# MoeinSorkhei/APLA

Measured on NVIDIA B200. Metric: ViT-B/14 APLA fine-tune images/sec/GPU at 1/2/4/8 B200; % bf16 tensor roofline, higher is better.
Workload: dtype bf16

## Files before the change

apla_b200/csrc/attention.cu:

```cuda
#include <cstdlib>

#include "common.cuh"
#include "kernels.cuh"
#include "ptx.cuh"

namespace apla {

namespace {

__global__ void attn_delta_kernel(const __nv_bfloat16* __restrict__ dout, const __nv_bfloat16* __restrict__ out,
                                  float* __restrict__ delta, size_t n_chunks) {
  const size_t i = size_t(blockIdx.x) * blockDim.x + threadIdx.x;
  float acc = 0.f;
  if (i < n_chunks) {
    const uint4 a = __ldg(reinterpret_cast<const uint4*>(dout) + i);
    const uint4 b = __ldg(reinterpret_cast<const uint4*>(out) + i);
    const uint32_t aw[4] = {a.x, a.y, a.z, a.w}, bw[4] = {b.x, b.y, b.z, b.w};
#pragma unroll
    for (int t = 0; t < 4; ++t) acc += bf16_lo(aw[t]) * bf16_lo(bw[t]) + bf16_hi(aw[t]) * bf16_hi(bw[t]);
  }
  acc += __shfl_xor_sync(0xffffffffu, acc, 1);
  acc += __shfl_xor_sync(0xffffffffu, acc, 2);
  acc += __shfl_xor_sync(0xffffffffu, acc, 4);
  if ((threadIdx.x & 7) == 0 && i < n_chunks) delta[i >> 3] = acc;
}

}

int attn_fwd(const void* qkv, void* out, float* lse, const int* cu_seqlens, int num_seqs, int max_seqlen,
             int total_tokens, int H,
             float scale, cudaStream_t stream) {
  APLA_CHECK(num_seqs > 0 && max_seqlen > 0 && H > 0, "attn_fwd: empty problem");
  if (attn_fused_supported(max_seqlen))
    return attn_fwd_sr(qkv, out, lse, cu_seqlens, num_seqs, max_seqlen, total_tokens, H, scale, stream);
  return attn_fwd_tc(qkv, out, lse, cu_seqlens, num_seqs, max_seqlen, total_tokens, H, scale, stream);
}

int attn_bwd(const void* qkv, const void* out, const void* dout, const float* lse, float* delta, void* dqkv,
             const int* cu_seqlens, int num_seqs, int max_seqlen, int total_tokens, int H, float scale,
             cudaStream_t stream) {
  APLA_CHECK(num_seqs > 0 && max_seqlen > 0 && H > 0, "attn_bwd: empty problem");
  if (out != nullptr) {
    const size_t n_chunks = size_t(total_tokens) * H * 8;
    attn_delta_kernel<<<(unsigned)((n_chunks + 255) / 256), 256, 0, stream>>>(
        reinterpret_cast<const __nv_bfloat16*>(dout), reinterpret_cast<const __nv_bfloat16*>(out), delta, n_chunks);
    APLA_CUDA(cudaGetLastError());
    count_launch();
  }
  static const bool v1 = [] { const char* e = getenv("APLA_ATTN_BWD_V1"); return e && atoi(e) != 0; }();
  if (!v1 && attn_bwd2_supported(max_seqlen))
    return attn_bwd2(qkv, dout, lse, delta, dqkv, cu_seqlens, num_seqs, max_seqlen, total_tokens, H, scale, stream);
  if (attn_fused_supported(max_seqlen))
    return attn_bwd_fused(qkv, dout, lse, delta, dqkv, cu_seqlens, num_seqs, max_seqlen, total_tokens, H, scale, stream);
  return attn_bwd_tc(qkv, dout, lse, delta, dqkv, cu_seqlens, num_seqs, max_seqlen, total_tokens, H, scale, stream);
}

}
```

apla_b200/csrc/attention_bwd2.cu:

```cuda
#include <cstdlib>

#include "common.cuh"
#include "kernels.cuh"
#include "ptx.cuh"

namespace apla {
namespace afb {

constexpr float LOG2E = 1.4426950408889634f;
constexpr int NT_MAX = 256;
constexpr int CW = 64;
constexpr int MAX_CHUNKS = NT_MAX / CW;
constexpr int kThreads = 640;
constexpr uint32_t RES_BYTES = NT_MAX * 128;
constexpr uint32_t TILE_BYTES = 128 * 128;
constexpr uint32_t OFF_Q = 0, OFF_DO = RES_BYTES, OFF_KV = 2 * RES_BYTES;
constexpr uint32_t OFF_DS = OFF_KV + 4 * TILE_BYTES;
constexpr uint32_t OFF_STAT = OFF_DS + 4 * TILE_BYTES;
constexpr uint32_t OFF_VEC = OFF_STAT + 2 * NT_MAX * 4;
constexpr uint32_t OFF_COL = OFF_VEC + 2 * 4 * 64 * 4;
constexpr uint32_t OFF_ROW = OFF_COL + 2 * 2 * NT_MAX * 4;
constexpr uint32_t OFF_PART = OFF_ROW + 2 * 2 * 128 * 4;
constexpr uint32_t OFF_BAR = OFF_PART + 4 * 3 * 64 * 4;
constexpr uint32_t SMEM_BYTES = OFF_BAR + 512 + 1024;
constexpr uint32_t TM_DQ = 0, TM_DK = 128, TM_DV = 192, TM_S = 256, TM_DP = 384, TM_COLS = 512;
static_assert(SMEM_BYTES <= 227 * 1024, "shared memory budget");

constexpr int REG_LAUNCH = 96;
constexpr int REG_WG0 = 56, REG_COMPUTE = 136, REG_EPI = 80, REG_HELP = 72;
static_assert(REG_WG0 + 2 * REG_COMPUTE + REG_EPI + REG_HELP <= 5 * REG_LAUNCH, "setmaxnreg budget exceeds the CTA's pool");

__device__ __forceinline__ void tmem_st_32x16(uint32_t taddr, const uint32_t (&v)[16]) {
  asm volatile(
      "tcgen05.st.sync.aligned.32x32b.x16.b32 [%0], {%1, %2, %3, %4, %5, %6, %7, %8, %9, %10, %11, %12, %13, %14, %15, %16};" ::
          "r"(taddr),
      "r"(v[0]), "r"(v[1]), "r"(v[2]), "r"(v[3]), "r"(v[4]), "r"(v[5]), "r"(v[6]), "r"(v[7]), "r"(v[8]), "r"(v[9]),
      "r"(v[10]), "r"(v[11]), "r"(v[12]), "r"(v[13]), "r"(v[14]), "r"(v[15])
      : "memory");
}
__device__ __forceinline__ void tmem_st_wait() { asm volatile("tcgen05.wait::st.sync.aligned;" ::: "memory"); }
__device__ __forceinline__ bool mbar_test(uint64_t* bar, uint32_t parity) {
  uint32_t ok;
  asm volatile(
      "{\n\t.reg .pred p;\n\t"
      "mbarrier.test_wait.parity.shared::cta.b64 p, [%1], %2;\n\t"
      "selp.u32 %0, 1, 0, p;\n\t}"
      : "=r"(ok)
      : "r"(smem_u32(bar)), "r"(parity)
      : "memory");
  return ok != 0;
}

constexpr uint32_t DESC_HI = (1024u >> 4) | (1u << 14) | (2u << 29);
constexpr uint32_t DESC_LO_K = (16u >> 4) << 16;
constexpr uint32_t DESC_LO_MN = (16384u >> 4) << 16;

__device__ __forceinline__ void umma_ss(uint32_t tmem_d, uint32_t a_lo, uint32_t b_lo, uint32_t idesc, uint32_t accumulate) {
  asm volatile(
      "{\n\t.reg .pred p;\n\t.reg .b64 da, db;\n\t"
      "setp.ne.b32 p, %4, 0;\n\t"
      "mov.b64 da, {%1, %5};\n\t"
      "mov.b64 db, {%2, %5};\n\t"
      "tcgen05.mma.cta_group::1.kind::f16 [%0], da, db, %3, p;\n\t}" ::"r"(tmem_d),
      "r"(a_lo), "r"(b_lo), "r"(idesc), "r"(accumulate), "r"(DESC_HI)
      : "memory");
}
__device__ __forceinline__ void umma_ts(uint32_t tmem_d, uint32_t tmem_a, uint32_t b_lo, uint32_t idesc, uint32_t accumulate) {
  asm volatile(
      "{\n\t.reg .pred p;\n\t.reg .b64 db;\n\t"
      "setp.ne.b32 p, %4, 0;\n\t"
      "mov.b64 db, {%2, %5};\n\t"
      "tcgen05.mma.cta_group::1.kind::f16 [%0], [%1], db, %3, p;\n\t}" ::"r"(tmem_d),
      "r"(tmem_a), "r"(b_lo), "r"(idesc), "r"(accumulate), "r"(DESC_HI)
      : "memory");
}

#ifdef APLA_AFB_DEBUG
__device__ __forceinline__ void wait_tag(uint64_t* bar, uint32_t parity, int tag) {
  uint32_t spins = 0;
  while (!mbar_try_wait(bar, parity)) {
    if (++spins > (1u << 16)) {
      if ((threadIdx.x & 31) == 0)
        printf("afb HANG cta %d warp %d tag %d parity %u\n", blockIdx.x, threadIdx.x >> 5, tag, parity);
// ... 108 lines not shown
    b0 = fmaf(bf16_lo(xb.z), q1.x, b0);
    b1 = fmaf(bf16_hi(xb.z), q1.y, b1);
    a0 = fmaf(bf16_lo(xa.w), p1.z, a0);
    a1 = fmaf(bf16_hi(xa.w), p1.w, a1);
    b0 = fmaf(bf16_lo(xb.w), q1.z, b0);
    b1 = fmaf(bf16_hi(xb.w), q1.w, b1);
  }
  da = a0 + a1;
  db = b0 + b1;
}
__device__ __forceinline__ float dot_vec64(uint32_t a, uint32_t b) {
  float s0 = 0.f, s1 = 0.f;
#pragma unroll 4
  for (int u = 0; u < 16; ++u) {
    const float4 x = lds_f4(a + 16 * u);
    const float4 y = lds_f4(b + 16 * u);
    s0 = fmaf(x.x, y.x, s0);
    s1 = fmaf(x.y, y.y, s1);
    s0 = fmaf(x.z, y.z, s0);
    s1 = fmaf(x.w, y.w, s1);
  }
  return s0 + s1;
}

__device__ __forceinline__ void drain_row64(uint32_t taddr, float mul, bool rank1, float coef, uint32_t vec,
                                            __nv_bfloat16* dst, bool store) {
  uint32_t pk[32];
#pragma unroll
  for (int c = 0; c < 2; ++c) {
    uint32_t ov[32];
    tmem_ld_32x32(taddr + c * 32, ov);
    tmem_ld_wait();
    if (rank1) {
#pragma unroll
      for (int i = 0; i < 8; ++i) {
        const float4 v = lds_f4(vec + (c * 32 + 4 * i) * 4);
        ov[4 * i + 0] = __float_as_uint(fmaf(coef, v.x, __uint_as_float(ov[4 * i + 0])));
        ov[4 * i + 1] = __float_as_uint(fmaf(coef, v.y, __uint_as_float(ov[4 * i + 1])));
        ov[4 * i + 2] = __float_as_uint(fmaf(coef, v.z, __uint_as_float(ov[4 * i + 2])));
        ov[4 * i + 3] = __float_as_uint(fmaf(coef, v.w, __uint_as_float(ov[4 * i + 3])));
      }
    }
#pragma unroll
    for (int i = 0; i < 16; ++i)
      pk[c * 16 + i] = pack_bf16(__uint_as_float(ov[2 * i]) * mul, __uint_as_float(ov[2 * i + 1]) * mul);
  }
  if (store) {
    uint4* d4 = reinterpret_cast<uint4*>(dst);
#pragma unroll
    for (int j = 0; j < 8; ++j) d4[j] = make_uint4(pk[4 * j], pk[4 * j + 1], pk[4 * j + 2], pk[4 * j + 3]);
  }
}

__global__ void __launch_bounds__(kThreads, 1)
attn_bwd2_kernel(const __grid_constant__ Maps maps, const __nv_bfloat16* __restrict__ qkv,
                 const __nv_bfloat16* __restrict__ dout, const float* __restrict__ lse, const float* __restrict__ delta,
                 __nv_bfloat16* __restrict__ dqkv, const int* __restrict__ cu_seqlens, int n_fixed, int H, int G,
                 float scale, int ablate) {
#ifndef APLA_AFB_ABLATE
  ablate = 0;
#endif
  extern __shared__ uint8_t smem_raw[];
  uint8_t* smem = reinterpret_cast<uint8_t*>((reinterpret_cast<uintptr_t>(smem_raw) + 1023) & ~uintptr_t(1023));
  uint64_t* bars = reinterpret_cast<uint64_t*>(smem + OFF_BAR);
  uint64_t* qdo_full = bars;
  uint64_t* qdo_empty = bars + 4;
  uint64_t* kv_full = bars + 8;
  uint64_t* kv_empty = bars + 10;
  uint64_t* s_full = bars + 12;
  uint64_t* s_free = bars + 14;
  uint64_t* dp_full = bars + 16;
  uint64_t* pd_full = bars + 18;
  uint64_t* ds_empty = bars + 20;
  uint64_t* acc_full = bars + 22;
  uint64_t* acc_empty = bars + 23;
  uint64_t* dq_full = bars + 24;
  uint64_t* dq_empty = bars + 25;
  uint64_t* hrow_full = bars + 26;
  uint64_t* hrow_empty = bars + 28;
  uint64_t* hcol_full = bars + 30;
  uint64_t* hcol_empty = bars + 32;
  uint64_t* pk_full = bars + 34;
  uint32_t* tmem_slot = reinterpret_cast<uint32_t*>(bars + 38);

  const int warp = __shfl_sync(0xffffffffu, threadIdx.x >> 5, 0), lane = threadIdx.x & 31;
  const Problem prob{cu_seqlens, n_fixed, H, G, (ablate & 2) != 0};
  const int D = H * 64;

  if (warp == 0 && lane == 0) {
    tma_prefetch_desc(&maps.qkv64);
    tma_prefetch_desc(&maps.qkv16);
    tma_prefetch_desc(&maps.do64);
    tma_prefetch_desc(&maps.do16);
    for (int i = 0; i < MAX_CHUNKS; ++i) {
      mbar_init(&qdo_full[i], 2);
      mbar_init(&qdo_empty[i], 4);
    }
    for (int i = 0; i < 2; ++i) {
      mbar_init(&kv_full[i], 1);
      mbar_init(&kv_empty[i], 4);
      mbar_init(&s_full[i], 1);
      mbar_init(&s_free[i], 4);
      mbar_init(&dp_full[i], 1);
      mbar_init(&pd_full[i], 4);
      mbar_init(&ds_empty[i], 1);
      mbar_init(&hrow_full[i], 1);
      mbar_init(&hrow_empty[i], 4);
      mbar_init(&hcol_full[i], 1);
      mbar_init(&hcol_empty[i], 4);
    }
    for (int i = 0; i < 4; ++i) mbar_init(&pk_full[i], 4);
    mbar_init(acc_full, 2);
    mbar_init(acc_empty, 4);
    mbar_init(dq_full, 1);
    mbar_init(dq_empty, 4);
    fence_barrier_init();
  }
  if (warp == 1) {
    tmem_alloc<1>(tmem_slot, TM_COLS);
    tmem_relinquish<1>();
  }
  tc_fence_before();
  __syncthreads();
  tc_fence_after();
  const uint32_t tmem = __shfl_sync(0xffffffffu, *tmem_slot, 0);
#ifdef APLA_AFB_PROF
  uint32_t prof[20];
#pragma unroll
  for (int i = 0; i < 20; ++i) prof[i] = 0;
  const long long prof_t0 = clock64();
#endif

#ifdef APLA_AFB_TRACE
  __shared__ long long tr_buf[6][200];
  __shared__ int tr_n[6];
  __shared__ long long tr_t0s;
  if (threadIdx.x == 0) {
    for (int i = 0; i < 6; ++i) tr_n[i] = 0;
    tr_t0s = clock64();
  }
  __syncthreads();
  const long long tr_t0 = tr_t0s;
#define TR(role, ev, arg)                                                                              \
  do {                                                                                                 \
    if (blockIdx.x == 0 && lane == 0 && tr_n[role] < 200)                                              \
      tr_buf[role][tr_n[role]++] = ((clock64() - tr_t0) << 16) | ((long long)(ev) << 8) | ((arg) & 255); \
  } while (0)
#else
#define TR(role, ev, arg)
#endif
  const uint32_t sb = smem_u32(smem);
  const uint32_t a_sl = sb + OFF_STAT, a_sd = a_sl + NT_MAX * 4;
  const uint32_t a_vec = sb + OFF_VEC;
  const uint32_t a_col = sb + OFF_COL;
  const uint32_t a_row = sb + OFF_ROW;

  if (warp < 4) {
    reg_dealloc<REG_WG0>();
    const bool leader = elect_one();
    const uint32_t q_lo = smem_u32(smem + OFF_Q) >> 4, do_lo = smem_u32(smem + OFF_DO) >> 4;
    const uint32_t kv_lo = smem_u32(smem + OFF_KV) >> 4, ds_lo = smem_u32(smem + OFF_DS) >> 4;
    if (warp == 0) {
      auto load_rows = [&](uint8_t* dst, const CUtensorMap* m64, const CUtensorMap* m16, uint64_t* bar, int col, int row,
                           int rows) {
        int r = 0;
        for (; r + 64 <= rows; r += 64) tma_load_2d(dst + r * 128, m64, bar, col, row + r);
// ... 109 lines not shown
        bool ok = true;
        if (w.jt == 0) ok = mbar_test(&qdo_full[w.j], (w.qpar >> w.j) & 1);
        if (ok && w.j == 0) ok = mbar_test(&kv_full[w.ts & 1], (w.ts >> 1) & 1);
        return __all_sync(0xffffffffu, ok) != 0;
      };
      Walk pc, dc;
      pc.init(prob);
      dc = pc;
      while (!dc.done(prob)) {
        while (!pc.done(prob) && pc.c <= dc.c) {
          wait_operands(pc);
          issue_dp(pc);
          pc.next_chunk(prob);
        }
        if (!pc.done(prob) && pc.c - dc.c < 2 && operands_ready(pc)) {
          tc_fence_after();
          issue_dp(pc);
          pc.next_chunk(prob);
        }
        const int slot = dc.ts & 1;
        WAIT(&pd_full[dc.c & 1], (dc.c >> 1) & 1, 8);
        if (dc.j == 0) WAIT(acc_empty, (dc.ts & 1) ^ 1, 9);
        tc_fence_after();
        const int n_k = (dc.valid_cols() + 15) >> 4;
        const uint32_t b_do = DESC_LO_MN + do_lo + dc.j * (CW * 128 >> 4);
        const uint32_t t_p = tmem + TM_DP + (dc.c & 1) * CW;
        TR(0, 4, dc.c);
        if (leader) {
#pragma unroll
          for (int kk = 0; kk < CW / 16; ++kk)
            if (kk < n_k) umma_ts(tmem + TM_DV, t_p + kk * 8, b_do + kk * 128, idesc_acc, (dc.j > 0 || kk > 0) ? 1u : 0u);
          if (dc.last_tile()) umma_commit(&qdo_empty[dc.j]);
          if (dc.last_chunk()) {
            umma_commit(acc_full);
            umma_commit(&kv_empty[slot]);
          }
        }
        __syncwarp();
        dc.next_chunk(prob);
        while (!pc.done(prob) && pc.c - dc.c < 2 && operands_ready(pc)) {
          tc_fence_after();
          issue_dp(pc);
          pc.next_chunk(prob);
        }
      }
    } else {
      const uint32_t idesc_acc = make_idesc_bf16(128, 64, 0, 1);
      const uint32_t idesc_dq = make_idesc_bf16(128, 64, 1, 1);
      Walk a;
      a.init(prob);
      while (!a.done(prob)) {
        const int slot = a.ts & 1;
        WAIT(&pk_full[a.c & 3], (a.c >> 2) & 1, 10);
        if (a.j == 0) WAIT(acc_empty, (a.ts & 1) ^ 1, 11);
        tc_fence_after();
        const int n_k = (a.valid_cols() + 15) >> 4;
        const int tq = a.tq();
        const uint32_t a_ds = DESC_LO_K + ds_lo + ((tq & 1) * 2 + (a.j & 1)) * (TILE_BYTES >> 4);
        const uint32_t b_q = DESC_LO_MN + q_lo + a.j * (CW * 128 >> 4);
        TR(0, 5, a.c);
        if (leader) {
#pragma unroll
          for (int kk = 0; kk < CW / 16; ++kk)
            if (kk < n_k && !(ablate & 16)) umma_ss(tmem + TM_DK, a_ds + 2 * kk, b_q + kk * 128, idesc_acc, (a.j > 0 || kk > 0) ? 1u : 0u);
          if (a.last_tile()) umma_commit(&qdo_empty[a.j]);
        }
        __syncwarp();
        if ((a.j & 1) || a.last_chunk()) {
          const int t = a.j >> 1;
          if (a.jt == 0 && t == 0) {
            WAIT(dq_empty, (a.gi & 1) ^ 1, 12);
            tc_fence_after();
          }
          const int n_kk = (a.valid_keys() + 15) >> 4;
          const uint32_t a_pair = DESC_LO_MN + ds_lo + (tq & 1) * (2 * TILE_BYTES >> 4);
          const uint32_t b_k = DESC_LO_MN + kv_lo + slot * (2 * TILE_BYTES >> 4);
          if (leader) {
#pragma unroll
            for (int kk = 0; kk < 8; ++kk)
              if (kk < n_kk && !(ablate & 16))
                umma_ss(tmem + TM_DQ + t * 64, a_pair + kk * 128, b_k + kk * 128, idesc_dq, (a.jt > 0 || kk > 0) ? 1u : 0u);
            umma_commit(&ds_empty[tq & 1]);
          }
          __syncwarp();
        }
        if (a.last_chunk()) {
          if (leader) {
            umma_commit(acc_full);
            umma_commit(&kv_empty[slot]);
            if (a.last_tile()) umma_commit(dq_full);
          }
          __syncwarp();
        }
        a.next_chunk(prob);
      }
    }
  } else if (warp < 12) {
    reg_alloc<REG_COMPUTE>();
    const int wg = (warp - 4) >> 2;
    const int quad = warp & 3;
    const int row = quad * 32 + lane;
    const uint32_t lane_addr = tmem + (uint32_t(quad * 32) << 16);
    const float sl2 = scale * LOG2E;
    const uint32_t sw = uint32_t(row & 7);
    Walk k;
    k.init(prob);
    while (!k.done(prob)) {
// ... 71 lines not shown
            pk[2 * i + 1] = pack_bf16(__uint_as_float(p0[4 * i + 2]) * (__uint_as_float(dv[4 * i + 2]) - d.z),
                                      __uint_as_float(p0[4 * i + 3]) * (__uint_as_float(dv[4 * i + 3]) - d.w));
          }
          CP(12);
          WAIT(&ds_empty[tq & 1], ((tq >> 1) & 1) ^ 1, 9);
          CP(19);
#pragma unroll
          for (int u = 0; u < 4; ++u) {
            uint4 val = make_uint4(pk[4 * u], pk[4 * u + 1], pk[4 * u + 2], pk[4 * u + 3]);
            if (!key_ok) val = make_uint4(0u, 0u, 0u, 0u);
            sts_u4(panel_row + ((uint32_t(u) ^ sw) << 4), val);
          }
#pragma unroll
          for (int i = 0; i < 16; ++i) pk[i] = pack_bf16(__uint_as_float(p0[2 * i]), __uint_as_float(p0[2 * i + 1]));
          tmem_st_32x16(t_dp, pk);
        }
        if (two) {
          uint32_t dv[32], pk[16];
          tmem_ld_32x32(t_dp + 32, dv);
          tmem_ld_wait();
#pragma unroll
          for (int i = 0; i < 8; ++i) {
            const float4 d = lds_f4(sD + 128 + 16 * i);
            pk[2 * i] = pack_bf16(__uint_as_float(p1[4 * i + 0]) * (__uint_as_float(dv[4 * i + 0]) - d.x),
                                  __uint_as_float(p1[4 * i + 1]) * (__uint_as_float(dv[4 * i + 1]) - d.y));
            pk[2 * i + 1] = pack_bf16(__uint_as_float(p1[4 * i + 2]) * (__uint_as_float(dv[4 * i + 2]) - d.z),
                                      __uint_as_float(p1[4 * i + 3]) * (__uint_as_float(dv[4 * i + 3]) - d.w));
          }
#pragma unroll
          for (int u = 0; u < 4; ++u) {
            uint4 val = make_uint4(pk[4 * u], pk[4 * u + 1], pk[4 * u + 2], pk[4 * u + 3]);
            if (!key_ok) val = make_uint4(0u, 0u, 0u, 0u);
            sts_u4(panel_row + ((uint32_t(4 + u) ^ sw) << 4), val);
          }
#pragma unroll
          for (int i = 0; i < 16; ++i) pk[i] = pack_bf16(__uint_as_float(p1[2 * i]), __uint_as_float(p1[2 * i + 1]));
          tmem_st_32x16(t_dp + 16, pk);
        }
        CP(13);
        tmem_st_wait();
        fence_proxy_async_smem();
        CP(14);
      }
      tc_fence_before();
      __syncwarp();
      if (lane == 0) {
        mbar_arrive(&pd_full[k.c & 1]);
        mbar_arrive(&pk_full[k.c & 3]);
      }
      if (quad == 0) TR(1 + wg, 5, k.c);
      k.next_chunk(prob);
    }
  } else if (warp < 16) {
    reg_dealloc<REG_EPI>();
    const int quad = warp & 3;
    const int row = quad * 32 + lane;
    const uint32_t lane_addr = tmem + (uint32_t(quad * 32) << 16);
    Walk k;
    k.init(prob);
    while (!k.done(prob)) {
      const int par = k.gi & 1, slot = k.ts & 1;
      const bool odd = k.odd != 0;
      const uint32_t vecs = a_vec + par * 1024;
      if (quad == 0) TR(3, 1, k.ts);
      WAIT(acc_full, k.ts & 1, 10);
      if (quad == 0) TR(3, 2, k.ts);
      tc_fence_after();
      WAIT(&hrow_full[slot], (k.ts >> 1) & 1, 11);
      if (quad == 0) TR(3, 3, k.ts);
      {
        const int r = k.jt * 128 + row;
        const bool ok = r < k.nt;
        __nv_bfloat16* base = dqkv + size_t(k.row_start + (ok ? r : 0)) * (3 * D) + k.h * 64;
        float cp = 0.f, cds = 0.f;
        if (odd) {
          cp = lds_f32(a_row + (slot * 256 + row) * 4);
          cds = lds_f32(a_row + (slot * 256 + 128 + row) * 4);
        }
        __syncwarp();
        if (lane == 0) mbar_arrive(&hrow_empty[slot]);
        if (!(ablate & 4))
        drain_row64(lane_addr + TM_DK, scale, odd, cds, vecs, base + D, ok);
        {
          uint32_t pk[32];
#pragma unroll
          for (int c = 0; c < 2; ++c) {
            uint32_t ov[32];
            if (!(ablate & 4)) {
              tmem_ld_32x32(lane_addr + TM_DV + c * 32, ov);
              tmem_ld_wait();
            }
            if (c == 1) {
              tc_fence_before();
              __syncwarp();
              if (lane == 0) mbar_arrive(acc_empty);
            }
            if (odd) {
#pragma unroll
              for (int i = 0; i < 8; ++i) {
                const float4 v = lds_f4(vecs + (192 + c * 32 + 4 * i) * 4);
                ov[4 * i + 0] = __float_as_uint(fmaf(cp, v.x, __uint_as_float(ov[4 * i + 0])));
                ov[4 * i + 1] = __float_as_uint(fmaf(cp, v.y, __uint_as_float(ov[4 * i + 1])));
                ov[4 * i + 2] = __float_as_uint(fmaf(cp, v.z, __uint_as_float(ov[4 * i + 2])));
                ov[4 * i + 3] = __float_as_uint(fmaf(cp, v.w, __uint_as_float(ov[4 * i + 3])));
              }
            }
#pragma unroll
            for (int i = 0; i < 16; ++i)
              pk[c * 16 + i] = pack_bf16(__uint_as_float(ov[2 * i]), __uint_as_float(ov[2 * i + 1]));
          }
          if (ok && !(ablate & 4)) {
            uint4* d4 = reinterpret_cast<uint4*>(base + 2 * D);
#pragma unroll
            for (int j = 0; j < 8; ++j) d4[j] = make_uint4(pk[4 * j], pk[4 * j + 1], pk[4 * j + 2], pk[4 * j + 3]);
          }
        }
      }
      if (k.last_tile()) {
        WAIT(dq_full, k.gi & 1, 12);
        tc_fence_after();
        WAIT(&hcol_full[par], (k.gi >> 1) & 1, 13);
        for (int t = 0; t < k.ntiles; ++t) {
          const int r = t * 128 + row;
          const bool ok = r < k.nt;
          __nv_bfloat16* base = dqkv + size_t(k.row_start + (ok ? r : 0)) * (3 * D) + k.h * 64;
          const float cq = odd ? lds_f32(a_col + (par * 512 + 256 + r) * 4) : 0.f;
          if (!(ablate & 4))
          drain_row64(lane_addr + TM_DQ + t * 64, scale, odd, cq, vecs + 64 * 4, base, ok);
        }
        tc_fence_before();
        __syncwarp();
        if (lane == 0) {
          mbar_arrive(dq_empty);
          mbar_arrive(&hcol_empty[par]);
        }
      }
      if (quad == 0) TR(3, 4, k.ts);
      const int ts0 = k.ts;
      while (!k.done(prob) && k.ts == ts0) k.next_chunk(prob);
    }
  } else {
    reg_dealloc<REG_HELP>();
    const int e = threadIdx.x - 512;
    const int dpair = e & 31, part = e >> 5;
    const float sl2 = scale * LOG2E;
    const uint32_t a_part = sb + OFF_PART;
    const uint32_t dp_off = (uint32_t(dpair & 3) << 2);
#ifdef APLA_AFB_PROF
    long long hp_t = clock64();
#define HP(i) do { const long long _n = clock64(); prof[i] += uint32_t(_n - hp_t); hp_t = _n; } while (0)
#else
#define HP(i)
#endif
    Walk k;
    k.init(prob);
    int ts = 0;
    while (!k.done(prob)) {
      HP(0);
      const int par = k.gi & 1;
      const bool odd = k.odd != 0;
      const int o = k.nt;
      const uint32_t vecs = a_vec + par * 1024, cols = a_col + par * 2048;
      WAIT(&hcol_empty[par], ((k.gi >> 1) & 1) ^ 1, 14);
      float lse2_o = 0.f, delta_o = 0.f;
      if (odd) {
        const int v = e >> 5;
        const size_t tok = size_t(k.row_start + o);
        const __nv_bfloat16* src = v < 3 ? qkv + tok * (3 * D) + v * D + k.h * 64 : dout + tok * D + k.h * 64;
        const uint32_t w2 = __ldg(reinterpret_cast<const uint32_t*>(src) + lane);
        sts_f32(vecs + (v * 64 + 2 * lane) * 4, bf16_lo(w2));
        sts_f32(vecs + (v * 64 + 2 * lane + 1) * 4, bf16_hi(w2));
        lse2_o = __ldg(lse + tok * H + k.h) * LOG2E;
        delta_o = __ldg(delta + tok * H + k.h);
      }
      HP(1);
      for (int j = 0; j < k.nchunks; ++j) WAIT(&qdo_full[j], (k.qpar >> j) & 1, 15);
      asm volatile("bar.sync 2, 128;" ::: "memory");
      HP(0);
      float p_oo = 0.f, ds_oo = 0.f;
      float ko0 = 0.f, ko1 = 0.f, vo0 = 0.f, vo1 = 0.f;
      if (odd) {
        const float s_oo = dot_vec64(vecs, vecs + 64 * 4), dp_oo = dot_vec64(vecs + 192 * 4, vecs + 128 * 4);
        p_oo = exp2f(fmaf(s_oo, sl2, -lse2_o));
        ds_oo = p_oo * (dp_oo - delta_o);
#pragma unroll
        for (int qq = 0; qq < 2; ++qq) {
          const int q = e + 128 * qq;
          float p = 0.f, ds = 0.f;
          if (q < k.nt) {
            float s, dp;
            dot2_row64(sb + OFF_Q + q * 128, sb + OFF_DO + q * 128, q, vecs + 64 * 4, vecs + 128 * 4, s, dp);
            p = exp2f(fmaf(s, sl2, -lds_f32(a_sl + q * 4)));
            ds = p * (dp - lds_f32(a_sd + q * 4));
          }
          sts_f32(cols + q * 4, p);
// ... 87 lines not shown
      k.next_group(prob);
    }
  }
#ifdef APLA_AFB_PROF
  if (blockIdx.x == 0 && lane == 0 && (warp == 4 || warp == 8 || warp == 5))
    printf("afb compute warp %d phases: S-load %u exps %u dP-load+dS-half0 %u stores+half1 %u st-wait+fence %u\n", warp, prof[10], prof[11],
           prof[12], prof[13], prof[14]);
  if (blockIdx.x == 0 && lane == 0 && warp == 16)
    printf("afb helper phases: other/waits %u vec-load %u col %u dk-loop %u tile-dots %u dq-loop %u finalize %u\n", prof[0], prof[1],
           prof[2], prof[3], prof[4], prof[5], prof[6]);
  if (blockIdx.x == 0 && lane == 0 && (warp <= 2 || (warp & 3) == 0) && warp != 16)
    printf("afb prof warp %2d total %lld | kv_empty %u qdo_empty %u acc_empty %u dq_empty %u qdo_empty(st) %u | qdo_full %u s_full %u "
           "dp_full %u ds_empty %u | acc_full %u hrow_full %u dq_full %u hcol_full %u | hcol_empty %u qdo_full(h) %u kv_full(h) %u "
           "hrow_empty %u | idle-spin %u issued %u\n",
           warp, clock64() - prof_t0, prof[1], prof[2], prof[3], prof[4], prof[5], prof[6], prof[7], prof[8], prof[9], prof[10],
           prof[11], prof[12], prof[13], prof[14], prof[15], prof[16], prof[17], prof[18], prof[19]);
#endif
  __syncwarp();
  tc_fence_before();
  __syncthreads();
#ifdef APLA_AFB_TRACE
  if (blockIdx.x == 0 && threadIdx.x == 0) {
    const char* names[5] = {"issuer", "wg0", "wg1", "epi", "producer"};
    for (int r = 0; r < 5; ++r) {
      printf("afbtrace %s:", names[r]);
      for (int i = 0; i < tr_n[r]; ++i)
        printf(" %lld.%lld@%lld", (tr_buf[r][i] >> 8) & 255, tr_buf[r][i] & 255, tr_buf[r][i] >> 16);
      printf("\n");
    }
  }
#endif
  if (warp == 1) {
    tc_fence_after();
    tmem_dealloc<1>(tmem, TM_COLS);
  }
}

}

bool attn_bwd2_supported(int max_seqlen) { return max_seqlen > 0 && max_seqlen <= afb::NT_MAX + 1; }

int attn_bwd2(const void* qkv, const void* dout, const float* lse, const float* delta, void* dqkv,
              const int* cu_seqlens, int num_seqs, int max_seqlen, int total_tokens, int H, float scale,
              cudaStream_t stream) {
  using namespace afb;
  APLA_CHECK(attn_bwd2_supported(max_seqlen), "attn_bwd2: max_seqlen %d exceeds the resident limit", max_seqlen);
  const int D = H * 64;
  const uint64_t T = total_tokens;
  Maps m;
  if (int rc = make_tmap_2d(&m.qkv64, qkv, 2, T, 3 * D, 3 * D, 64, 64, true)) return rc;
  if (int rc = make_tmap_2d(&m.qkv16, qkv, 2, T, 3 * D, 3 * D, 16, 64, true)) return rc;
  if (int rc = make_tmap_2d(&m.do64, dout, 2, T, D, D, 64, 64, true)) return rc;
  if (int rc = make_tmap_2d(&m.do16, dout, 2, T, D, D, 16, 64, true)) return rc;
  static bool attr_set = false;
  if (!attr_set) {
    APLA_CUDA(cudaFuncSetAttribute(attn_bwd2_kernel, cudaFuncAttributeMaxDynamicSharedMemorySize, (int)SMEM_BYTES));
    attr_set = true;
  }
  const int G = num_seqs * H;
  const int grid = G < sm_count() ? G : sm_count();
  int ablate = 0;
#ifdef APLA_AFB_ABLATE
  if (const char* e = getenv("APLA_AFB_ABLATE")) ablate = atoi(e);
#endif
  attn_bwd2_kernel<<<grid, kThreads, SMEM_BYTES, stream>>>(
      m, reinterpret_cast<const __nv_bfloat16*>(qkv), reinterpret_cast<const __nv_bfloat16*>(dout), lse, delta,
      reinterpret_cast<__nv_bfloat16*>(dqkv), cu_seqlens, max_seqlen, H, G, scale, ablate);
  APLA_CUDA(cudaGetLastError());
  count_launch();
  return 0;
}

}
```

apla_b200/csrc/kernels.cuh:

```cuda
#pragma once
#include <cuda_runtime.h>
#include <stdint.h>

namespace apla {

enum { EPI_BIAS = 0, EPI_BIAS_GELU = 1, EPI_RESID = 2, EPI_GELU_BWD = 3, EPI_F32_T = 4, EPI_DELTA = 5, EPI_BIAS_GELU_D = 6,
       EPI_MUL_F16 = 7, EPI_RED = 8, EPI_RESID_LN = 9, EPI_BIAS_GELU_G = 10, EPI_RESID_SCALED = 11 };

int gemm_tn(int epi, const void* A, const void* B, int M, int N, int K, int lda, int ldb, void* out, void* out2,
            const float* bias, const float* gamma, const void* aux, int ldo, cudaStream_t stream, int bn_override);
int gemm2_tn(int epi, const void* A, const void* B, int M, int N, int K, int lda, int ldb, void* out, void* out2,
             const float* bias, const float* gamma, const void* aux, int ldo, cudaStream_t stream, int bn);
int gemm_wgrad_nt(const void* A, const void* B, int M, int N, int K, int lda, int ldb, float* dW, int ldw,
                  const int* rowmap, int n_valid, cudaStream_t stream);
int gemm_resid_ln(const void* A, const void* B, int M, int N, int K, int lda, int ldb, float* out, const float* bias,
                  const float* gamma, const float* resid, int ldo, const float* ln_w, const float* ln_b, void* ln_out,
                  int ld_ln, float eps, cudaStream_t stream, int fuse_mode = -1, const float* row_scale = nullptr,
                  int rows_per_scale = 1);
int gemm_resid_scaled(const void* A, const void* B, int M, int N, int K, int lda, int ldb, float* out, const float* bias,
                      const float* gamma, const float* resid, int ldo, const float* row_scale, int rows_per_scale,
                      cudaStream_t stream);
int gemm2_resid_scaled(const void* A, const void* B, int M, int N, int K, int lda, int ldb, float* out, const float* bias,
                       const float* gamma, const float* resid, int ldo, const float* row_scale, int rows_per_scale,
                       cudaStream_t stream, int bn);
bool gemm2_resid_ln_supported(int N);
int gemm2_resid_ln(const void* A, const void* B, int M, int N, int K, int lda, int ldb, float* out, const float* bias,
                   const float* gamma, const float* resid, int ldo, const float* ln_w, const float* ln_b, void* ln_out,
                   int ld_ln, float eps, cudaStream_t stream);

int attn_fwd(const void* qkv, void* out, float* lse, const int* cu_seqlens, int num_seqs, int max_seqlen,
             int total_tokens, int H,
             float scale, cudaStream_t stream);
int attn_fwd_tc(const void* qkv, void* out, float* lse, const int* cu_seqlens, int num_seqs, int max_seqlen,
                int total_tokens, int H, float scale, cudaStream_t stream);
int attn_bwd_tc(const void* qkv, const void* dout, const float* lse, const float* delta, void* dqkv,
                const int* cu_seqlens, int num_seqs, int max_seqlen, int total_tokens, int H, float scale,
                cudaStream_t stream);
int attn_fwd_sr(const void* qkv, void* out, float* lse, const int* cu_seqlens, int num_seqs, int max_seqlen,
                int total_tokens, int H, float scale, cudaStream_t stream);
bool attn_fused_supported(int max_seqlen);
int attn_bwd_fused(const void* qkv, const void* dout, const float* lse, const float* delta, void* dqkv,
                   const int* cu_seqlens, int num_seqs, int max_seqlen, int total_tokens, int H, float scale,
                   cudaStream_t stream);
bool attn_bwd2_supported(int max_seqlen);
int attn_bwd2(const void* qkv, const void* dout, const float* lse, const float* delta, void* dqkv,
              const int* cu_seqlens, int num_seqs, int max_seqlen, int total_tokens, int H, float scale,
              cudaStream_t stream);
int attn_bwd(const void* qkv, const void* out, const void* dout, const float* lse, float* delta, void* dqkv,
             const int* cu_seqlens, int num_seqs, int max_seqlen, int total_tokens, int H, float scale,
             cudaStream_t stream);

int attn_cls_fwd(const void* qkv, void* out, float* lse, int B, int N, int H, float scale, cudaStream_t stream);
int attn_cls_bwd(const void* qkv, const void* out, const void* dout, const float* lse, void* dqkv, int B, int N, int H,
                 float scale, cudaStream_t stream);

int attn_probs(const void* qkv, const float* lse, float* probs, int B, int N, int H, int q_rows, float scale,
               cudaStream_t stream);

int layernorm_fwd(const float* x, int64_t ldx, const float* w, const float* b, void* y, int64_t ldy, int rows, int D,
                  float eps, cudaStream_t stream);
int layernorm_bwd(const void* dy, int64_t ld_dy, const float* x, int64_t ldx, const float* w, const float* dres,
                  int64_t ld_dres, float* dx, int64_t ld_dx, void* dxb, int64_t ld_dxb, const float* gamma, void* sub,
                  int64_t ld_sub, const int* idx, int r, int r_pad, int rows, int D, float eps, cudaStream_t stream,
                  const float* row_scale = nullptr, int rows_per_scale = 1);
int gather_cols(const void* dy, int64_t ld, void* sub, int64_t ld_sub, const int* idx, int r, int r_pad, int rows,
                cudaStream_t stream);
int ls_cast(const float* x, int64_t ldx, const float* gamma, void* out, int64_t ldo, int rows, int D,
            cudaStream_t stream);
int colsum(const void* a, int64_t ld, int rows, int n, float* out, const int* rowmap, cudaStream_t stream);
int patchify(const float* img, void* out, int B, int S, int p, int kpad, cudaStream_t stream);
int assemble_tokens(const void* patch, const float* cls, const float* pos, float* x, int B, int P, int D,
                    cudaStream_t stream);

int head_fwd(const void* xn, const float* W, const float* bias, float* logits, int B, int D, int C, cudaStream_t s);
int cross_entropy(const float* logits, const int64_t* labels, float* dlogits, float* loss, int B, int C,
                  float grad_scale, float loss_scale, cudaStream_t s);
int cross_entropy_soft(const float* logits, const float* targets, float* dlogits, float* loss, int B, int C,
                       float grad_scale, float loss_scale, cudaStream_t s);
int eval_accumulate(const float* logits, const int64_t* labels, int B, int C, float* acc, cudaStream_t s);
int bce_with_logits(const float* logits, const float* targets, float* dlogits, float* loss, int B, int C,
                    float grad_scale, float loss_scale, cudaStream_t s);
int eval_accumulate_bce(const float* logits, const float* targets, int B, int C, double* acc, cudaStream_t s);
int head_bwd(const float* dlogits, const void* xn, const float* W, float* dW, float* db, void* dxn, int B, int D, int C,
             cudaStream_t s);
int grad_sumsq(const float* g, int64_t n, float scale, float* out, cudaStream_t s);
int adamw_step(float* p, const float* g, float* m, float* v, int64_t n, int64_t n_decay, const float* sumsq,
               float gscale, float max_norm, float lr, float wd, float b1, float b2, float eps, int step,
               cudaStream_t s, const float* hyper = nullptr);
int proj_refresh(const float* w1, const float* b1, const int* idx, void* wfull, void* wfullT, float* bfull, int L,
                 int r, int D, int64_t w1_block_stride, int64_t b1_block_stride, cudaStream_t s);
// ... 45 lines not shown
```

Measured before the change: 7937.

## Release dV/dK accumulators early in attention backward epilogue with separate dK barrier

The attention backward epilogue warps now load the dV accumulator from tensor memory first and release it straight away. dK is read next and freed through a new dk_empty barrier, which the MMA warp waits on before starting the next dK/dV accumulation, so tensor-core work can overlap the bf16 packing and global stores. Registers move from the helper warps to the epilogue warps to hold the 64-column row buffers. The previous epilogue stays available behind an environment variable through a templated kernel. The risk is register pressure in the epilogue and lost helper-warp throughput.

```diff
diff --git a/apla_b200/csrc/attention.cu b/apla_b200/csrc/attention.cu
--- a/apla_b200/csrc/attention.cu
+++ b/apla_b200/csrc/attention.cu
@@ -25,6 +25,11 @@
   if ((threadIdx.x & 7) == 0 && i < n_chunks) delta[i >> 3] = acc;
 }
 
+}
+
+bool attn_epi_v1() {
+  static const bool v1 = [] { const char* e = getenv("APLA_ATTN_EPI_V1"); return e && atoi(e) != 0; }();
+  return v1;
 }
 
 int attn_fwd(const void* qkv, void* out, float* lse, const int* cu_seqlens, int num_seqs, int max_seqlen,
diff --git a/apla_b200/csrc/attention_bwd2.cu b/apla_b200/csrc/attention_bwd2.cu
--- a/apla_b200/csrc/attention_bwd2.cu
+++ b/apla_b200/csrc/attention_bwd2.cu
@@ -27,8 +27,10 @@
 static_assert(SMEM_BYTES <= 227 * 1024, "shared memory budget");
 
 constexpr int REG_LAUNCH = 96;
-constexpr int REG_WG0 = 56, REG_COMPUTE = 136, REG_EPI = 80, REG_HELP = 72;
+constexpr int REG_WG0 = 56, REG_COMPUTE = 136, REG_EPI = 88, REG_HELP = 64;
+constexpr int REG_EPI_V1 = 80, REG_HELP_V1 = 72;
 static_assert(REG_WG0 + 2 * REG_COMPUTE + REG_EPI + REG_HELP <= 5 * REG_LAUNCH, "setmaxnreg budget exceeds the CTA's pool");
+static_assert(REG_WG0 + 2 * REG_COMPUTE + REG_EPI_V1 + REG_HELP_V1 <= 5 * REG_LAUNCH, "setmaxnreg budget exceeds the CTA's pool");
 
 __device__ __forceinline__ void tmem_st_32x16(uint32_t taddr, const uint32_t (&v)[16]) {
   asm volatile(
@@ -243,6 +245,43 @@
   }
 }
 
+__device__ __forceinline__ void load_row64(uint32_t taddr, uint32_t (&v)[4][16]) {
+#pragma unroll
+  for (int q = 0; q < 4; ++q) tmem_ld_32x16(taddr + q * 16, v[q]);
+  tmem_ld_wait();
+}
+template <bool SCALED>
+__device__ __forceinline__ void finish_row64(uint32_t (&v)[4][16], float mul, bool rank1, float coef, uint32_t vec,
+                                             __nv_bfloat16* dst, bool store) {
+#pragma unroll
+  for (int c = 0; c < 2; ++c) {
+    if (rank1) {
+#pragma unroll
+      for (int i = 0; i < 8; ++i) {
+        const float4 x = lds_f4(vec + (c * 32 + 4 * i) * 4);
+        uint32_t* o = &v[2 * c + (i >> 2)][(i & 3) * 4];
+        o[0] = __float_as_uint(fmaf(coef, x.x, __uint_as_float(o[0])));
+        o[1] = __float_as_uint(fmaf(coef, x.y, __uint_as_float(o[1])));
+        o[2] = __float_as_uint(fmaf(coef, x.z, __uint_as_float(o[2])));
+        o[3] = __float_as_uint(fmaf(coef, x.w, __uint_as_float(o[3])));
+      }
+    }
+    uint32_t pk[16];
+#pragma unroll
+    for (int i = 0; i < 16; ++i) {
+      const float a = __uint_as_float(v[2 * c + (i >> 3)][(2 * i) & 15]);
+      const float b = __uint_as_float(v[2 * c + (i >> 3)][(2 * i + 1) & 15]);
+      pk[i] = SCALED ? pack_bf16(a * mul, b * mul) : pack_bf16(a, b);
+    }
+    if (store) {
+      uint4* d4 = reinterpret_cast<uint4*>(dst) + c * 4;
+#pragma unroll
+      for (int j = 0; j < 4; ++j) d4[j] = make_uint4(pk[4 * j], pk[4 * j + 1], pk[4 * j + 2], pk[4 * j + 3]);
+    }
+  }
+}
+
+template <bool kDefer>
 __global__ void __launch_bounds__(kThreads, 1)
 attn_bwd2_kernel(const __grid_constant__ Maps maps, const __nv_bfloat16* __restrict__ qkv,
                  const __nv_bfloat16* __restrict__ dout, const float* __restrict__ lse, const float* __restrict__ delta,
@@ -272,7 +311,8 @@
   uint64_t* hcol_full = bars + 30;
   uint64_t* hcol_empty = bars + 32;
   uint64_t* pk_full = bars + 34;
-  uint32_t* tmem_slot = reinterpret_cast<uint32_t*>(bars + 38);
+  uint64_t* dk_empty = bars + 38;
+  uint32_t* tmem_slot = reinterpret_cast<uint32_t*>(bars + 40);
 
   const int warp = __shfl_sync(0xffffffffu, threadIdx.x >> 5, 0), lane = threadIdx.x & 31;
   const Problem prob{cu_seqlens, n_fixed, H, G, (ablate & 2) != 0};
@@ -303,6 +343,7 @@
     for (int i = 0; i < 4; ++i) mbar_init(&pk_full[i], 4);
     mbar_init(acc_full, 2);
     mbar_init(acc_empty, 4);
+    mbar_init(dk_empty, 4);
     mbar_init(dq_full, 1);
     mbar_init(dq_empty, 4);
     fence_barrier_init();
@@ -518,7 +559,7 @@
       while (!a.done(prob)) {
         const int slot = a.ts & 1;
         WAIT(&pk_full[a.c & 3], (a.c >> 2) & 1, 10);
-        if (a.j == 0) WAIT(acc_empty, (a.ts & 1) ^ 1, 11);
+        if (a.j == 0) WAIT(kDefer ? dk_empty : acc_empty, (a.ts & 1) ^ 1, 11);
         tc_fence_after();
         const int n_k = (a.valid_cols() + 15) >> 4;
         const int tq = a.tq();
@@ -696,7 +737,7 @@
       k.next_chunk(prob);
     }
   } else if (warp < 16) {
-    reg_dealloc<REG_EPI>();
+    reg_dealloc<kDefer ? REG_EPI : REG_EPI_V1>();
     const int quad = warp & 3;
     const int row = quad * 32 + lane;
     const uint32_t lane_addr = tmem + (uint32_t(quad * 32) << 16);
@@ -707,15 +748,20 @@
       const bool odd = k.odd != 0;
       const uint32_t vecs = a_vec + par * 1024;
       if (quad == 0) TR(3, 1, k.ts);
-      WAIT(acc_full, k.ts & 1, 10);
-      if (quad == 0) TR(3, 2, k.ts);
-      tc_fence_after();
-      WAIT(&hrow_full[slot], (k.ts >> 1) & 1, 11);
-      if (quad == 0) TR(3, 3, k.ts);
-      {
+      if (kDefer) {
         const int r = k.jt * 128 + row;
-        const bool ok = r < k.nt;
-        __nv_bfloat16* base = dqkv + size_t(k.row_start + (ok ? r : 0)) * (3 * D) + k.h * 64;
+        const bool ok = r < k.nt && !(ablate & 4);
+        __nv_bfloat16* base = dqkv + size_t(k.row_start + (r < k.nt ? r : 0)) * (3 * D) + k.h * 64;
+        WAIT(acc_full, k.ts & 1, 10);
+        if (quad == 0) TR(3, 2, k.ts);
+        tc_fence_after();
+        uint32_t v[4][16];
+        if (!(ablate & 4)) load_row64(lane_addr + TM_DV, v);
+        tc_fence_before();
+        __syncwarp();
+        if (lane == 0) mbar_arrive(acc_empty);
+        WAIT(&hrow_full[slot], (k.ts >> 1) & 1, 11);
+        if (quad == 0) TR(3, 3, k.ts);
         float cp = 0.f, cds = 0.f;
         if (odd) {
           cp = lds_f32(a_row + (slot * 256 + row) * 4);
@@ -723,60 +769,104 @@
         }
         __syncwarp();
         if (lane == 0) mbar_arrive(&hrow_empty[slot]);
-        if (!(ablate & 4))
-        drain_row64(lane_addr + TM_DK, scale, odd, cds, vecs, base + D, ok);
-        {
-          uint32_t pk[32];
-#pragma unroll
-          for (int c = 0; c < 2; ++c) {
-            uint32_t ov[32];
-            if (!(ablate & 4)) {
-              tmem_ld_32x32(lane_addr + TM_DV + c * 32, ov);
-              tmem_ld_wait();
-            }
-            if (c == 1) {
+        finish_row64<false>(v, 1.f, odd, cp, vecs + 192 * 4, base + 2 * D, ok);
+        if (!(ablate & 4)) load_row64(lane_addr + TM_DK, v);
+        tc_fence_before();
+        __syncwarp();
+        if (lane == 0) mbar_arrive(dk_empty);
+        finish_row64<true>(v, scale, odd, cds, vecs, base + D, ok);
+        if (k.last_tile()) {
+          WAIT(dq_full, k.gi & 1, 12);
+          tc_fence_after();
+          for (int t = 0; t < k.ntiles; ++t) {
+            const int rq = t * 128 + row;
+            const bool okq = rq < k.nt && !(ablate & 4);
+            __nv_bfloat16* bq = dqkv + size_t(k.row_start + (rq < k.nt ? rq : 0)) * (3 * D) + k.h * 64;
+            if (!(ablate & 4)) load_row64(lane_addr + TM_DQ + t * 64, v);
+            if (t == k.ntiles - 1) {
               tc_fence_before();
               __syncwarp();
-              if (lane == 0) mbar_arrive(acc_empty);
+              if (lane == 0) mbar_arrive(dq_empty);
             }
-            if (odd) {
-#pragma unroll
-              for (int i = 0; i < 8; ++i) {
-                const float4 v = lds_f4(vecs + (192 + c * 32 + 4 * i) * 4);
-                ov[4 * i + 0] = __float_as_uint(fmaf(cp, v.x, __uint_as_float(ov[4 * i + 0])));
-                ov[4 * i + 1] = __float_as_uint(fmaf(cp, v.y, __uint_as_float(ov[4 * i + 1])));
-                ov[4 * i + 2] = __float_as_uint(fmaf(cp, v.z, __uint_as_float(ov[4 * i + 2])));
-                ov[4 * i + 3] = __float_as_uint(fmaf(cp, v.w, __uint_as_float(ov[4 * i + 3])));
-              }
-            }
-#pragma unroll
-            for (int i = 0; i < 16; ++i)
-              pk[c * 16 + i] = pack_bf16(__uint_as_float(ov[2 * i]), __uint_as_float(ov[2 * i + 1]));
-          }
-          if (ok && !(ablate & 4)) {
-            uint4* d4 = reinterpret_cast<uint4*>(base + 2 * D);
-#pragma unroll
-            for (int j = 0; j < 8; ++j) d4[j] = make_uint4(pk[4 * j], pk[4 * j + 1], pk[4 * j + 2], pk[4 * j + 3]);
-          }
-        }
-      }
-      if (k.last_tile()) {
-        WAIT(dq_full, k.gi & 1, 12);
+            if (t == 0) WAIT(&hcol_full[par], (k.gi >> 1) & 1, 13);
+            const float cq = odd ? lds_f32(a_col + (par * 512 + 256 + rq) * 4) : 0.f;
+            finish_row64<true>(v, scale, odd, cq, vecs + 64 * 4, bq, okq);
+          }
+          __syncwarp();
+          if (lane == 0) mbar_arrive(&hcol_empty[par]);
+        }
+      } else {
+        WAIT(acc_full, k.ts & 1, 10);
+        if (quad == 0) TR(3, 2, k.ts);
         tc_fence_after();
-        WAIT(&hcol_full[par], (k.gi >> 1) & 1, 13);
-        for (int t = 0; t < k.ntiles; ++t) {
-          const int r = t * 128 + row;
+        WAIT(&hrow_full[slot], (k.ts >> 1) & 1, 11);
+        if (quad == 0) TR(3, 3, k.ts);
+        {
+          const int r = k.jt * 128 + row;
           const bool ok = r < k.nt;
           __nv_bfloat16* base = dqkv + size_t(k.row_start + (ok ? r : 0)) * (3 * D) + k.h * 64;
-          const float cq = odd ? lds_f32(a_col + (par * 512 + 256 + r) * 4) : 0.f;
+          float cp = 0.f, cds = 0.f;
+          if (odd) {
+            cp = lds_f32(a_row + (slot * 256 + row) * 4);
+            cds = lds_f32(a_row + (slot * 256 + 128 + row) * 4);
+          }
+          __syncwarp();
+          if (lane == 0) mbar_arrive(&hrow_empty[slot]);
           if (!(ablate & 4))
-          drain_row64(lane_addr + TM_DQ + t * 64, scale, odd, cq, vecs + 64 * 4, base, ok);
-        }
-        tc_fence_before();
-        __syncwarp();
-        if (lane == 0) {
-          mbar_arrive(dq_empty);
-          mbar_arrive(&hcol_empty[par]);
+          drain_row64(lane_addr + TM_DK, scale, odd, cds, vecs, base + D, ok);
+          {
+            uint32_t pk[32];
+  #pragma unroll
+            for (int c = 0; c < 2; ++c) {
+              uint32_t ov[32];
+              if (!(ablate & 4)) {
+                tmem_ld_32x32(lane_addr + TM_DV + c * 32, ov);
+                tmem_ld_wait();
+              }
+              if (c == 1) {
+                tc_fence_before();
+                __syncwarp();
+                if (lane == 0) mbar_arrive(acc_empty);
+              }
+              if (odd) {
+  #pragma unroll
+                for (int i = 0; i < 8; ++i) {
+                  const float4 v = lds_f4(vecs + (192 + c * 32 + 4 * i) * 4);
+                  ov[4 * i + 0] = __float_as_uint(fmaf(cp, v.x, __uint_as_float(ov[4 * i + 0])));
+                  ov[4 * i + 1] = __float_as_uint(fmaf(cp, v.y, __uint_as_float(ov[4 * i + 1])));
+                  ov[4 * i + 2] = __float_as_uint(fmaf(cp, v.z, __uint_as_float(ov[4 * i + 2])));
+                  ov[4 * i + 3] = __float_as_uint(fmaf(cp, v.w, __uint_as_float(ov[4 * i + 3])));
+                }
+              }
+  #pragma unroll
+              for (int i = 0; i < 16; ++i)
+                pk[c * 16 + i] = pack_bf16(__uint_as_float(ov[2 * i]), __uint_as_float(ov[2 * i + 1]));
+            }
+            if (ok && !(ablate & 4)) {
+              uint4* d4 = reinterpret_cast<uint4*>(base + 2 * D);
+  #pragma unroll
+              for (int j = 0; j < 8; ++j) d4[j] = make_uint4(pk[4 * j], pk[4 * j + 1], pk[4 * j + 2], pk[4 * j + 3]);
+            }
+          }
+        }
+        if (k.last_tile()) {
+          WAIT(dq_full, k.gi & 1, 12);
+          tc_fence_after();
+          WAIT(&hcol_full[par], (k.gi >> 1) & 1, 13);
+          for (int t = 0; t < k.ntiles; ++t) {
+            const int r = t * 128 + row;
+            const bool ok = r < k.nt;
+            __nv_bfloat16* base = dqkv + size_t(k.row_start + (ok ? r : 0)) * (3 * D) + k.h * 64;
+            const float cq = odd ? lds_f32(a_col + (par * 512 + 256 + r) * 4) : 0.f;
+            if (!(ablate & 4))
+            drain_row64(lane_addr + TM_DQ + t * 64, scale, odd, cq, vecs + 64 * 4, base, ok);
+          }
+          tc_fence_before();
+          __syncwarp();
+          if (lane == 0) {
+            mbar_arrive(dq_empty);
+            mbar_arrive(&hcol_empty[par]);
+          }
         }
       }
       if (quad == 0) TR(3, 4, k.ts);
@@ -784,7 +874,7 @@
       while (!k.done(prob) && k.ts == ts0) k.next_chunk(prob);
     }
   } else {
-    reg_dealloc<REG_HELP>();
+    reg_dealloc<kDefer ? REG_HELP : REG_HELP_V1>();
     const int e = threadIdx.x - 512;
     const int dpair = e & 31, part = e >> 5;
     const float sl2 = scale * LOG2E;
@@ -978,10 +1068,11 @@
   if (int rc = make_tmap_2d(&m.qkv16, qkv, 2, T, 3 * D, 3 * D, 16, 64, true)) return rc;
   if (int rc = make_tmap_2d(&m.do64, dout, 2, T, D, D, 64, 64, true)) return rc;
   if (int rc = make_tmap_2d(&m.do16, dout, 2, T, D, D, 16, 64, true)) return rc;
-  static bool attr_set = false;
-  if (!attr_set) {
-    APLA_CUDA(cudaFuncSetAttribute(attn_bwd2_kernel, cudaFuncAttributeMaxDynamicSharedMemorySize, (int)SMEM_BYTES));
-    attr_set = true;
+  auto kernel = attn_epi_v1() ? attn_bwd2_kernel<false> : attn_bwd2_kernel<true>;
+  static bool attr_set[2] = {false, false};
+  if (!attr_set[attn_epi_v1()]) {
+    APLA_CUDA(cudaFuncSetAttribute(kernel, cudaFuncAttributeMaxDynamicSharedMemorySize, (int)SMEM_BYTES));
+    attr_set[attn_epi_v1()] = true;
   }
   const int G = num_seqs * H;
   const int grid = G < sm_count() ? G : sm_count();
@@ -989,7 +1080,7 @@
 #ifdef APLA_AFB_ABLATE
   if (const char* e = getenv("APLA_AFB_ABLATE")) ablate = atoi(e);
 #endif
-  attn_bwd2_kernel<<<grid, kThreads, SMEM_BYTES, stream>>>(
+  kernel<<<grid, kThreads, SMEM_BYTES, stream>>>(
       m, reinterpret_cast<const __nv_bfloat16*>(qkv), reinterpret_cast<const __nv_bfloat16*>(dout), lse, delta,
       reinterpret_cast<__nv_bfloat16*>(dqkv), cu_seqlens, max_seqlen, H, G, scale, ablate);
   APLA_CUDA(cudaGetLastError());
diff --git a/apla_b200/csrc/kernels.cuh b/apla_b200/csrc/kernels.cuh
--- a/apla_b200/csrc/kernels.cuh
+++ b/apla_b200/csrc/kernels.cuh
@@ -36,6 +36,7 @@
 int attn_bwd_tc(const void* qkv, const void* dout, const float* lse, const float* delta, void* dqkv,
                 const int* cu_seqlens, int num_seqs, int max_seqlen, int total_tokens, int H, float scale,
                 cudaStream_t stream);
+bool attn_epi_v1();
 int attn_fwd_sr(const void* qkv, void* out, float* lse, const int* cu_seqlens, int num_seqs, int max_seqlen,
                 int total_tokens, int H, float scale, cudaStream_t stream);
 bool attn_fused_supported(int max_seqlen);
```

Result: faster. 8142 (median of 6 runs) (+2.6%).
